# nagadomi/nunif

Hardware: NVIDIA H100
Metric: waifu2x_input_megapixels_per_sec (higher is better)
Workload: dtype f16

## Files before the change

nunif_b200/csrc/gemm_wgmma.cuh:

```cuda
#pragma once
#include "common.cuh"
#include "ptx.cuh"
#include <cuda.h>

namespace nb200 {

enum : int { ACT_NONE = 0, ACT_LRELU01 = 1, ACT_GELU = 2, ACT_RELU = 3 };
enum : int { OUT_NHWC = 0, OUT_PIXSHUF2 = 1, OUT_SPLIT = 2 };

struct GemmParams {
    int B, Ho, Wo, TH, TW, tiles_x, tiles_y;
    int N;
    int taps, cpt;
    int8_t tap_dx[16], tap_dy[16], tap_dyi[16];
    int n_tiles;
    const float* bias;
    int act;
    int out_mode, cout;
    int has_res, res_cy, res_cx;
    int res_before_act;
    int k2;
};

struct GemmMaps {
    CUtensorMap a, b;
    CUtensorMap o[4];
    union {
        CUtensorMap r[4];
        CUtensorMap a2;
    };
};

__device__ __forceinline__ void mbar_init(uint64_t* bar, uint32_t count) {
    asm volatile("mbarrier.init.shared::cta.b64 [%0], %1;" ::"r"(smem_u32(bar)), "r"(count));
}
__device__ __forceinline__ void mbar_expect_tx(uint64_t* bar, uint32_t bytes) {
    asm volatile("mbarrier.arrive.expect_tx.shared::cta.b64 _, [%0], %1;" ::"r"(smem_u32(bar)), "r"(bytes) : "memory");
}
__device__ __forceinline__ void mbar_arrive(uint64_t* bar) {
    asm volatile("mbarrier.arrive.shared::cta.b64 _, [%0];" ::"r"(smem_u32(bar)) : "memory");
}
__device__ __forceinline__ void mbar_wait(uint64_t* bar, uint32_t parity) {
    const uint32_t addr = smem_u32(bar);
    uint32_t done = 0;
#pragma unroll 1
    for (uint32_t it = 0; it < (1u << 18) && !done; ++it)
        asm volatile(
            "{\n\t.reg .pred p;\n\t"
            "mbarrier.try_wait.parity.shared::cta.b64 p, [%1], %2, %3;\n\t"
            "selp.u32 %0, 1, 0, p;\n\t}"
            : "=r"(done) : "r"(addr), "r"(parity), "r"(20000u) : "memory");
    if (!done) __trap();
}
__device__ __forceinline__ void fence_barrier_init() {
    asm volatile("fence.mbarrier_init.release.cluster;" ::: "memory");
    asm volatile("fence.proxy.async.shared::cta;" ::: "memory");
}
__device__ __forceinline__ void tma_load_5d(const CUtensorMap* map, uint64_t* bar, void* dst, int c0, int c1, int c2, int c3, int c4) {
    asm volatile(
        "cp.async.bulk.tensor.5d.shared::cluster.global.tile.mbarrier::complete_tx::bytes [%0], [%1, {%3, %4, %5, %6, %7}], [%2];"
        ::"r"(smem_u32(dst)), "l"(map), "r"(smem_u32(bar)), "r"(c0), "r"(c1), "r"(c2), "r"(c3), "r"(c4) : "memory");
}
__device__ __forceinline__ void tma_load_2d(const CUtensorMap* map, uint64_t* bar, void* dst, int c0, int c1) {
    asm volatile(
        "cp.async.bulk.tensor.2d.shared::cluster.global.tile.mbarrier::complete_tx::bytes [%0], [%1, {%3, %4}], [%2];"
        ::"r"(smem_u32(dst)), "l"(map), "r"(smem_u32(bar)), "r"(c0), "r"(c1) : "memory");
}
__device__ __forceinline__ void tma_load_4d(const CUtensorMap* map, uint64_t* bar, void* dst, int c0, int c1, int c2, int c3) {
    asm volatile(
        "cp.async.bulk.tensor.4d.shared::cluster.global.tile.mbarrier::complete_tx::bytes [%0], [%1, {%3, %4, %5, %6}], [%2];"
        ::"r"(smem_u32(dst)), "l"(map), "r"(smem_u32(bar)), "r"(c0), "r"(c1), "r"(c2), "r"(c3) : "memory");
}
__device__ __forceinline__ void tma_store_4d(const CUtensorMap* map, const void* src, int c0, int c1, int c2, int c3) {
    asm volatile("cp.async.bulk.tensor.4d.global.shared::cta.tile.bulk_group [%0, {%2, %3, %4, %5}], [%1];"
                 ::"l"(map), "r"(smem_u32(src)), "r"(c0), "r"(c1), "r"(c2), "r"(c3) : "memory");
}
__device__ __forceinline__ void tma_store_2d(const CUtensorMap* map, const void* src, int c0, int c1) {
    asm volatile("cp.async.bulk.tensor.2d.global.shared::cta.tile.bulk_group [%0, {%2, %3}], [%1];"
                 ::"l"(map), "r"(smem_u32(src)), "r"(c0), "r"(c1) : "memory");
}
__device__ __forceinline__ void tma_store_commit() { asm volatile("cp.async.bulk.commit_group;" ::: "memory"); }
__device__ __forceinline__ void tma_store_wait_read() { asm volatile("cp.async.bulk.wait_group.read 0;" ::: "memory"); }
__device__ __forceinline__ void fence_async_smem() { asm volatile("fence.proxy.async.shared::cta;" ::: "memory"); }
__device__ __forceinline__ void consumer_bar_sync() { asm volatile("bar.sync 1, 256;" ::: "memory"); }
__device__ __forceinline__ void tma_prefetch_desc(const CUtensorMap* map) {
    asm volatile("prefetch.tensormap [%0];" ::"l"(map) : "memory");
}
__device__ __forceinline__ bool elect_one() {
    uint32_t pred;
    asm volatile(
        "{\n\t.reg .pred p;\n\t"
        "elect.sync _|p, 0xffffffff;\n\t"
        "selp.u32 %0, 1, 0, p;\n\t}"
        : "=r"(pred));
    return pred != 0;
}
__device__ __forceinline__ void wgmma_fence() { asm volatile("wgmma.fence.sync.aligned;" ::: "memory"); }
__device__ __forceinline__ void wgmma_commit() { asm volatile("wgmma.commit_group.sync.aligned;" ::: "memory"); }
template <int N>
__device__ __forceinline__ void wgmma_wait() { asm volatile("wgmma.wait_group.sync.aligned %0;" ::"n"(N) : "memory"); }
template <int K>
__device__ __forceinline__ void wgmma_fence_operands(float (&d)[K]) {
#pragma unroll
    for (int j = 0; j < K; ++j) asm volatile("" : "+f"(d[j])::"memory");
}

template <int SWIZZLE_BYTES>
__device__ __forceinline__ uint64_t make_kmajor_desc(uint32_t saddr) {
    constexpr uint64_t layout = SWIZZLE_BYTES == 128 ? 1 : (SWIZZLE_BYTES == 64 ? 2 : 3);
    constexpr uint64_t sbo = (8 * SWIZZLE_BYTES) >> 4;
    return (uint64_t)((saddr & 0x3FFFF) >> 4) | (1ull << 16) | (sbo << 32) | (layout << 62);
}

template <int N>
__device__ void wgmma_f16(float (&d)[N / 2], uint64_t a, uint64_t b, uint32_t acc);
template <> __device__ __forceinline__ void wgmma_f16<16>(float (&d)[8], uint64_t a, uint64_t b, uint32_t acc) {
    asm volatile("{\n\t.reg .pred p;\n\tsetp.ne.b32 p, %10, 0;\n\t"
                 "wgmma.mma_async.sync.aligned.m64n16k16.f32.f16.f16 {%0, %1, %2, %3, %4, %5, %6, %7}, %8, %9, p, 1, 1, 0, 0;\n\t}"
                 : "+f"(d[0]), "+f"(d[1]), "+f"(d[2]), "+f"(d[3]), "+f"(d[4]), "+f"(d[5]), "+f"(d[6]), "+f"(d[7])
                 : "l"(a), "l"(b), "r"(acc));
}
template <> __device__ __forceinline__ void wgmma_f16<32>(float (&d)[16], uint64_t a, uint64_t b, uint32_t acc) {
    asm volatile("{\n\t.reg .pred p;\n\tsetp.ne.b32 p, %18, 0;\n\t"
                 "wgmma.mma_async.sync.aligned.m64n32k16.f32.f16.f16 {%0, %1, %2, %3, %4, %5, %6, %7, %8, %9, %10, %11, %12, %13, %14, %15}, %16, %17, p, 1, 1, 0, 0;\n\t}"
                 : "+f"(d[0]), "+f"(d[1]), "+f"(d[2]), "+f"(d[3]), "+f"(d[4]), "+f"(d[5]), "+f"(d[6]), "+f"(d[7]), "+f"(d[8]), "+f"(d[9]), "+f"(d[10]), "+f"(d[11]), "+f"(d[12]), "+f"(d[13]), "+f"(d[14]), "+f"(d[15])
                 : "l"(a), "l"(b), "r"(acc));
}
template <> __device__ __forceinline__ void wgmma_f16<48>(float (&d)[24], uint64_t a, uint64_t b, uint32_t acc) {
    asm volatile("{\n\t.reg .pred p;\n\tsetp.ne.b32 p, %26, 0;\n\t"
                 "wgmma.mma_async.sync.aligned.m64n48k16.f32.f16.f16 {%0, %1, %2, %3, %4, %5, %6, %7, %8, %9, %10, %11, %12, %13, %14, %15, %16, %17, %18, %19, %20, %21, %22, %23}, %24, %25, p, 1, 1, 0, 0;\n\t}"
                 : "+f"(d[0]), "+f"(d[1]), "+f"(d[2]), "+f"(d[3]), "+f"(d[4]), "+f"(d[5]), "+f"(d[6]), "+f"(d[7]), "+f"(d[8]), "+f"(d[9]), "+f"(d[10]), "+f"(d[11]), "+f"(d[12]), "+f"(d[13]), "+f"(d[14]), "+f"(d[15]), "+f"(d[16]), "+f"(d[17]), "+f"(d[18]), "+f"(d[19]), "+f"(d[20]), "+f"(d[21]), "+f"(d[22]), "+f"(d[23])
                 : "l"(a), "l"(b), "r"(acc));
}
template <> __device__ __forceinline__ void wgmma_f16<64>(float (&d)[32], uint64_t a, uint64_t b, uint32_t acc) {
    asm volatile("{\n\t.reg .pred p;\n\tsetp.ne.b32 p, %34, 0;\n\t"
                 "wgmma.mma_async.sync.aligned.m64n64k16.f32.f16.f16 {%0, %1, %2, %3, %4, %5, %6, %7, %8, %9, %10, %11, %12, %13, %14, %15, %16, %17, %18, %19, %20, %21, %22, %23, %24, %25, %26, %27, %28, %29, %30, %31}, %32, %33, p, 1, 1, 0, 0;\n\t}"
                 : "+f"(d[0]), "+f"(d[1]), "+f"(d[2]), "+f"(d[3]), "+f"(d[4]), "+f"(d[5]), "+f"(d[6]), "+f"(d[7]), "+f"(d[8]), "+f"(d[9]), "+f"(d[10]), "+f"(d[11]), "+f"(d[12]), "+f"(d[13]), "+f"(d[14]), "+f"(d[15]), "+f"(d[16]), "+f"(d[17]), "+f"(d[18]), "+f"(d[19]), "+f"(d[20]), "+f"(d[21]), "+f"(d[22]), "+f"(d[23]), "+f"(d[24]), "+f"(d[25]), "+f"(d[26]), "+f"(d[27]), "+f"(d[28]), "+f"(d[29]), "+f"(d[30]), "+f"(d[31])
                 : "l"(a), "l"(b), "r"(acc));
}
template <> __device__ __forceinline__ void wgmma_f16<96>(float (&d)[48], uint64_t a, uint64_t b, uint32_t acc) {
    asm volatile("{\n\t.reg .pred p;\n\tsetp.ne.b32 p, %50, 0;\n\t"
                 "wgmma.mma_async.sync.aligned.m64n96k16.f32.f16.f16 {%0, %1, %2, %3, %4, %5, %6, %7, %8, %9, %10, %11, %12, %13, %14, %15, %16, %17, %18, %19, %20, %21, %22, %23, %24, %25, %26, %27, %28, %29, %30, %31, %32, %33, %34, %35, %36, %37, %38, %39, %40, %41, %42, %43, %44, %45, %46, %47}, %48, %49, p, 1, 1, 0, 0;\n\t}"
                 : "+f"(d[0]), "+f"(d[1]), "+f"(d[2]), "+f"(d[3]), "+f"(d[4]), "+f"(d[5]), "+f"(d[6]), "+f"(d[7]), "+f"(d[8]), "+f"(d[9]), "+f"(d[10]), "+f"(d[11]), "+f"(d[12]), "+f"(d[13]), "+f"(d[14]), "+f"(d[15]), "+f"(d[16]), "+f"(d[17]), "+f"(d[18]), "+f"(d[19]), "+f"(d[20]), "+f"(d[21]), "+f"(d[22]), "+f"(d[23]), "+f"(d[24]), "+f"(d[25]), "+f"(d[26]), "+f"(d[27]), "+f"(d[28]), "+f"(d[29]), "+f"(d[30]), "+f"(d[31]), "+f"(d[32]), "+f"(d[33]), "+f"(d[34]), "+f"(d[35]), "+f"(d[36]), "+f"(d[37]), "+f"(d[38]), "+f"(d[39]), "+f"(d[40]), "+f"(d[41]), "+f"(d[42]), "+f"(d[43]), "+f"(d[44]), "+f"(d[45]), "+f"(d[46]), "+f"(d[47])
                 : "l"(a), "l"(b), "r"(acc));
}
template <> __device__ __forceinline__ void wgmma_f16<128>(float (&d)[64], uint64_t a, uint64_t b, uint32_t acc) {
    asm volatile("{\n\t.reg .pred p;\n\tsetp.ne.b32 p, %66, 0;\n\t"
                 "wgmma.mma_async.sync.aligned.m64n128k16.f32.f16.f16 {%0, %1, %2, %3, %4, %5, %6, %7, %8, %9, %10, %11, %12, %13, %14, %15, %16, %17, %18, %19, %20, %21, %22, %23, %24, %25, %26, %27, %28, %29, %30, %31, %32, %33, %34, %35, %36, %37, %38, %39, %40, %41, %42, %43, %44, %45, %46, %47, %48, %49, %50, %51, %52, %53, %54, %55, %56, %57, %58, %59, %60, %61, %62, %63}, %64, %65, p, 1, 1, 0, 0;\n\t}"
                 : "+f"(d[0]), "+f"(d[1]), "+f"(d[2]), "+f"(d[3]), "+f"(d[4]), "+f"(d[5]), "+f"(d[6]), "+f"(d[7]), "+f"(d[8]), "+f"(d[9]), "+f"(d[10]), "+f"(d[11]), "+f"(d[12]), "+f"(d[13]), "+f"(d[14]), "+f"(d[15]), "+f"(d[16]), "+f"(d[17]), "+f"(d[18]), "+f"(d[19]), "+f"(d[20]), "+f"(d[21]), "+f"(d[22]), "+f"(d[23]), "+f"(d[24]), "+f"(d[25]), "+f"(d[26]), "+f"(d[27]), "+f"(d[28]), "+f"(d[29]), "+f"(d[30]), "+f"(d[31]), "+f"(d[32]), "+f"(d[33]), "+f"(d[34]), "+f"(d[35]), "+f"(d[36]), "+f"(d[37]), "+f"(d[38]), "+f"(d[39]), "+f"(d[40]), "+f"(d[41]), "+f"(d[42]), "+f"(d[43]), "+f"(d[44]), "+f"(d[45]), "+f"(d[46]), "+f"(d[47]), "+f"(d[48]), "+f"(d[49]), "+f"(d[50]), "+f"(d[51]), "+f"(d[52]), "+f"(d[53]), "+f"(d[54]), "+f"(d[55]), "+f"(d[56]), "+f"(d[57]), "+f"(d[58]), "+f"(d[59]), "+f"(d[60]), "+f"(d[61]), "+f"(d[62]), "+f"(d[63])
                 : "l"(a), "l"(b), "r"(acc));
}

__device__ __forceinline__ void wgmma_f16_rs96(float (&d)[48], const uint32_t (&a)[4], uint64_t b, uint32_t acc) {
    asm volatile("{\n\t.reg .pred p;\n\tsetp.ne.b32 p, %53, 0;\n\t"
                 "wgmma.mma_async.sync.aligned.m64n96k16.f32.f16.f16 {%0, %1, %2, %3, %4, %5, %6, %7, %8, %9, %10, %11, %12, %13, %14, %15, %16, %17, %18, %19, %20, %21, %22, %23, %24, %25, %26, %27, %28, %29, %30, %31, %32, %33, %34, %35, %36, %37, %38, %39, %40, %41, %42, %43, %44, %45, %46, %47}, {%48, %49, %50, %51}, %52, p, 1, 1, 0;\n\t}"
                 : "+f"(d[0]), "+f"(d[1]), "+f"(d[2]), "+f"(d[3]), "+f"(d[4]), "+f"(d[5]), "+f"(d[6]), "+f"(d[7]), "+f"(d[8]), "+f"(d[9]), "+f"(d[10]), "+f"(d[11]), "+f"(d[12]), "+f"(d[13]), "+f"(d[14]), "+f"(d[15]), "+f"(d[16]), "+f"(d[17]), "+f"(d[18]), "+f"(d[19]), "+f"(d[20]), "+f"(d[21]), "+f"(d[22]), "+f"(d[23]), "+f"(d[24]), "+f"(d[25]), "+f"(d[26]), "+f"(d[27]), "+f"(d[28]), "+f"(d[29]), "+f"(d[30]), "+f"(d[31]), "+f"(d[32]), "+f"(d[33]), "+f"(d[34]), "+f"(d[35]), "+f"(d[36]), "+f"(d[37]), "+f"(d[38]), "+f"(d[39]), "+f"(d[40]), "+f"(d[41]), "+f"(d[42]), "+f"(d[43]), "+f"(d[44]), "+f"(d[45]), "+f"(d[46]), "+f"(d[47])
                 : "r"(a[0]), "r"(a[1]), "r"(a[2]), "r"(a[3]), "l"(b), "r"(acc));
}

__device__ __forceinline__ float gelu_erf(float x) {
    const float a = fabsf(x);
    float q = fmaf(a, 4.88118734e-04f, -7.19881030e-03f);
    q = fmaf(q, a, 5.21468017e-02f);
    q = fmaf(q, a, 4.59595724e-01f);
    q = fmaf(q, a, 1.15100057e+00f);
    const float e = ex2(fmaf(-q, a, -1.0f));
    return fmaxf(x, 0.f) - a * e;
}

template <int K>
__device__ __forceinline__ void apply_act(float (&v)[K], int act) {
    switch (act) {
        case ACT_LRELU01:
#pragma unroll
            for (int j = 0; j < K; ++j) v[j] = v[j] > 0.f ? v[j] : 0.1f * v[j];
            break;
        case ACT_GELU:
#pragma unroll
            for (int j = 0; j < K; ++j) v[j] = gelu_erf(v[j]);
            break;
        case ACT_RELU:
#pragma unroll
            for (int j = 0; j < K; ++j) v[j] = fmaxf(v[j], 0.f);
            break;
        default: break;
    }
}

constexpr int GEMM_CONSUMER_THREADS = 256;
constexpr int GEMM_THREADS = GEMM_CONSUMER_THREADS + 32;

template <int BLOCK_N, int BK>
struct GemmCfg {
    static_assert(BLOCK_N % 16 == 0 && BLOCK_N <= 128, "BLOCK_N: 16..128 (the fp32 accumulators live in registers)");
    static constexpr int SWIZZLE = BK * 2;
    static constexpr int A_BYTES = 128 * BK * 2;
    static constexpr int B_BYTES = BLOCK_N * BK * 2;
    static constexpr int STAGE_BYTES = A_BYTES + ((B_BYTES + 1023) / 1024) * 1024;
    static constexpr int STAGES = (98304 / STAGE_BYTES) < 2 ? 2 : ((98304 / STAGE_BYTES) > 6 ? 6 : (98304 / STAGE_BYTES));
    static constexpr int CW = (BLOCK_N % 64 == 0) ? 64 : ((BLOCK_N % 32 == 0) ? 32 : 16);
    static constexpr int NCH = BLOCK_N / CW;
    static constexpr int CH_BYTES = 128 * CW * 2;
    static_assert(NCH * CH_BYTES <= STAGES * STAGE_BYTES, "epilogue staging must fit in the (drained) pipeline stages");
    static constexpr int SMEM_BYTES = STAGES * STAGE_BYTES + 1024  + 256 ;
};

template <int CW>
__device__ __forceinline__ uint32_t stage_off(int r, int j) {
    if (CW == 64) return (uint32_t)(r * 128 + ((j ^ (r & 7)) << 4));
    if (CW == 32) return (uint32_t)(r * 64 + ((j ^ ((r >> 1) & 3)) << 4));
    return (uint32_t)(r * 32 + ((j ^ ((r >> 2) & 1)) << 4));
}

template <int ROWS>
__device__ __forceinline__ uint32_t sw64_off(int r, int col) {
    return (uint32_t)((col >> 5) * (ROWS * 64)) + stage_off<32>(r, (col & 31) >> 3) + (uint32_t)((col & 7) * 2);
}

template <int BLOCK_N, int BK, bool A2 = false>
// ... 142 lines not shown
```

nunif_b200/csrc/swin_block.cu:

```cuda
#include "gemm_wgmma.cuh"
#include "swin_kernels.h"
#include "tmap.h"
#include <algorithm>

namespace nb200 {

extern int g_tune[16];

constexpr int FM_ROWS = 128, FM_STAGES = 5, FM_THREADS = GEMM_CONSUMER_THREADS + 128;
constexpr int FM_PRODUCER_REGS = 40, FM_CONSUMER_REGS = 232;

template <int C>
struct FmCfg {
    static constexpr int KB = C / 32;
    static constexpr int NBUF = C == 96 ? 3 : 2;
    static constexpr int TILE = FM_ROWS * C * 2;
    static constexpr int STAGE = 128 * C;
    static constexpr int SMEM = NBUF * TILE + FM_STAGES * STAGE + (2 * FM_STAGES + NBUF * (KB + 2) + 1) * 8 + 1024;
    static_assert(SMEM <= 232448, "shared memory per CTA exceeds the opt-in limit");
};

struct FmMaps {
    CUtensorMap x, att, wp, w1, w2, y, wy;
};

template <int K>
__device__ __forceinline__ float (&half96(float (&acc)[K], int h))[48] { return *reinterpret_cast<float(*)[48]>(&acc[48 * h]); }

__device__ __forceinline__ void wgmma_wait_n(int n) {
    if (n == 0) wgmma_wait<0>();
    else wgmma_wait<1>();
}

template <int C, bool PROJ, int CS>
__global__ void __launch_bounds__(FM_THREADS, 1) swin_mlp_fused_kernel(const __grid_constant__ FmMaps maps, const float* __restrict__ bp,
                                                                     const float* __restrict__ b1, const float* __restrict__ b2,
                                                                     const float* __restrict__ by, int ntiles) {
    using Cfg = FmCfg<C>;
    static_assert(CS % 16 == 0 && 2 * C * CS <= Cfg::STAGE && CS * 256 <= Cfg::TILE, "Wy must fit a ring stage, y a tile");
    constexpr int KB = Cfg::KB, NP = (KB + 1) / 2, NH = 2 * C / 64, NHALF = C / 96, NBUF = Cfg::NBUF;
    constexpr int SPT = (PROJ ? NP : 0) + 2 * NH + (CS ? 1 : 0);
    static_assert(SPT > FM_STAGES, "the barrier protocol needs more stages per tile than the ring holds");
    constexpr int XAHEAD = PROJ ? NBUF - 1 : NBUF;
    extern __shared__ uint8_t smem_dyn[];
    uint8_t* smem = smem_dyn + ((1024u - (smem_u32(smem_dyn) & 1023u)) & 1023u);
    uint8_t* ring = smem + NBUF * Cfg::TILE;
    uint64_t* full = reinterpret_cast<uint64_t*>(ring + FM_STAGES * Cfg::STAGE);
    uint64_t* empty = full + FM_STAGES;
    uint64_t* abar = empty + FM_STAGES;
    uint64_t* xbar = abar + NBUF * KB;
    uint64_t* outw = xbar + NBUF;
    uint64_t* xfree = outw + NBUF;
    auto buf = [&](int b) { return smem + b * Cfg::TILE; };
    const int tid = threadIdx.x, warp = tid >> 5;
    const int nt = (ntiles - (int)blockIdx.x + (int)gridDim.x - 1) / (int)gridDim.x;
    if (tid == GEMM_CONSUMER_THREADS) {
        tma_prefetch_desc(&maps.x);
        tma_prefetch_desc(&maps.w1);
        tma_prefetch_desc(&maps.w2);
        if (CS) {
            tma_prefetch_desc(&maps.wy);
            tma_prefetch_desc(&maps.y);
        }
        if (PROJ) {
            tma_prefetch_desc(&maps.att);
            tma_prefetch_desc(&maps.wp);
        }
        for (int s = 0; s < FM_STAGES; ++s) {
            mbar_init(&full[s], 1);
            mbar_init(&empty[s], 2);
        }
        for (int b = 0; b < NBUF; ++b) {
            for (int kb = 0; kb < KB; ++kb) mbar_init(&abar[b * KB + kb], 1);
            mbar_init(&xbar[b], 1);
            mbar_init(&outw[b], 2);
        }
        mbar_init(xfree, 2);
        fence_barrier_init();
    }
    __syncthreads();

    if (warp >= GEMM_CONSUMER_THREADS / 32) {
        asm volatile("setmaxnreg.dec.sync.aligned.u32 %0;" ::"n"(FM_PRODUCER_REGS));
        if (warp == GEMM_CONSUMER_THREADS / 32 && elect_one()) {
            int it = 0;
            auto push = [&](const CUtensorMap* m, int k0, int n0, int rows, int nbox) {
                const int s = it % FM_STAGES;
                mbar_wait(&empty[s], ((it / FM_STAGES) & 1) ^ 1);
                mbar_expect_tx(&full[s], nbox * rows * 64);
                for (int b = 0; b < nbox; ++b) tma_load_2d(m, &full[s], ring + s * Cfg::STAGE + b * rows * 64, k0 + 32 * b, n0);
                ++it;
            };
            for (int j = 0; j < nt; ++j) {
                if (PROJ)
                    for (int p = 0; p < NP; ++p) push(&maps.wp, 64 * p, 0, C, min(2, KB - 2 * p));
                push(&maps.w1, 0, 0, 64, KB);
                for (int hc = 0; hc < NH; ++hc) {
                    if (hc + 1 < NH) push(&maps.w1, 0, (hc + 1) * 64, 64, KB);
                    push(&maps.w2, hc * 64, 0, C, 2);
                }
                if (CS) push(&maps.wy, 0, 0, CS, KB);
            }
        } else if (warp == GEMM_CONSUMER_THREADS / 32 + 1 && elect_one()) {
            auto row = [&](int j) { return ((int)blockIdx.x + j * (int)gridDim.x) * FM_ROWS; };
            auto load_att = [&](int j) {
                const int b = j % NBUF;
                for (int kb = 0; kb < KB; ++kb) {
                    mbar_expect_tx(&abar[b * KB + kb], FM_ROWS * 64);
                    tma_load_2d(&maps.att, &abar[b * KB + kb], buf(b) + kb * (FM_ROWS * 64), kb * 32, row(j));
                }
            };
            auto load_x = [&](int j) {
                uint8_t* dst = buf((j + PROJ) % NBUF);
                mbar_expect_tx(&xbar[j % NBUF], Cfg::TILE);
                for (int kb = 0; kb < KB; ++kb) tma_load_2d(&maps.x, &xbar[j % NBUF], dst + kb * (FM_ROWS * 64), kb * 32, row(j));
            };
            asm volatile("griddepcontrol.wait;" ::: "memory");
            if (PROJ) load_att(0);
            for (int j = 0; j < XAHEAD && j < nt; ++j) load_x(j);
            for (int j = 0; j < nt; ++j) {
                if (PROJ) {
                    mbar_wait(xfree, j & 1);
                    if (j + 1 < nt) load_att(j + 1);
                }
                const int b = j % NBUF;
                mbar_wait(&outw[b], (j / NBUF) & 1);
                if constexpr (CS > 0)
                    for (int c = 0; c < CS / 16; ++c) tma_store_2d(&maps.y, buf(b) + c * (FM_ROWS * 32), 16 * c, row(j));
                else
                    for (int kb = 0; kb < KB; ++kb) tma_store_2d(&maps.x, buf(b) + kb * (FM_ROWS * 64), kb * 32, row(j));
                tma_store_commit();
                tma_store_wait_read();
                if (j + XAHEAD < nt) load_x(j + XAHEAD);
            }
        }
        return;
    }

    asm volatile("setmaxnreg.inc.sync.aligned.u32 %0;" ::"n"(FM_CONSUMER_REGS));
    const int wg = tid >> 7, t = tid & 127;
    const int row0 = wg * 64 + (t >> 5) * 16 + ((t & 31) >> 2);
    const int cq = 2 * (t & 3);
#pragma unroll 1
    for (int it0 = 0; (int)blockIdx.x + it0 / SPT * (int)gridDim.x < ntiles; it0 += SPT) {
        const int j = it0 / SPT;
        int it = it0;
        const int b = j % NBUF;
        const uint32_t par = (j / NBUF) & 1;
        uint8_t* sx1 = buf(b);
        const uint8_t* sxin = buf((j + PROJ) % NBUF);
        const uint32_t x1_base = smem_u32(sx1) + wg * 64 * 64;
        int pending = 0;
        auto take = [&]() -> uint32_t {
            const int s = it % FM_STAGES;
            mbar_wait(&full[s], (it / FM_STAGES) & 1);
            return smem_u32(ring + s * Cfg::STAGE);
        };
        auto commit = [&]() {
            wgmma_commit();
            ++it;
            ++pending;
        };
        auto retire = [&](int n) {
            wgmma_wait_n(n);
#pragma unroll
            for (int k = 0; k < FM_STAGES; ++k)
                if (k < pending - n && t == 0) mbar_arrive(&empty[(it - pending + k) % FM_STAGES]);
            pending = min(pending, n);
        };

        if (PROJ) {
            float acc[C / 2];
#pragma unroll
            for (int i = 0; i < C / 2; ++i) acc[i] = 0.f;
            wgmma_fence_operands(acc);
#pragma unroll
            for (int p = 0; p < NP; ++p) {
                const uint32_t bb = take();
#pragma unroll
                for (int kb = 2 * p; kb < 2 * p + 2 && kb < KB; ++kb) mbar_wait(&abar[b * KB + kb], par);
                wgmma_fence();
#pragma unroll
                for (int kb = 2 * p; kb < 2 * p + 2 && kb < KB; ++kb) {
                    const uint32_t a = x1_base + kb * (FM_ROWS * 64), w = bb + (kb - 2 * p) * (C * 64);
#pragma unroll
                    for (int s = 0; s < 2; ++s)
#pragma unroll
                        for (int h = 0; h < NHALF; ++h)
                            wgmma_f16<96>(half96(acc, h), make_kmajor_desc<64>(a + 32 * s), make_kmajor_desc<64>(w + h * 96 * 64 + 32 * s), 1u);
                }
                commit();
                retire(1);
            }
            retire(0);
            wgmma_fence_operands(acc);
            mbar_wait(&xbar[b], par);
#pragma unroll
            for (int q = 0; q < C / 8; ++q) {
                const int col = 8 * q + cq;
                const float2 bq = __ldg(reinterpret_cast<const float2*>(bp + col));
#pragma unroll
                for (int i = 0; i < 2; ++i) {
                    const uint32_t off = sw64_off<FM_ROWS>(row0 + 8 * i, col);
                    const float2 xv = __half22float2(*reinterpret_cast<const __half2*>(sxin + off));
                    *reinterpret_cast<__half2*>(sx1 + off) =
                        __floats2half2_rn(xv.x + (acc[4 * q + 2 * i] + bq.x), xv.y + (acc[4 * q + 2 * i + 1] + bq.y));
                }
            }
            fence_async_smem();
            asm volatile("bar.sync %0, 128;" ::"r"(2 + wg) : "memory");
            if (t == 0) mbar_arrive(xfree);
        } else {
            mbar_wait(&xbar[b], par);
        }

        float oacc[C / 2];
#pragma unroll
        for (int i = 0; i < C / 2; ++i) oacc[i] = 0.f;
        wgmma_fence_operands(oacc);
        float hacc[2][32];
        uint32_t af[4][4];
        auto fc1 = [&](float (&h)[32]) {
#pragma unroll
            for (int i = 0; i < 32; ++i) h[i] = 0.f;
            wgmma_fence_operands(h);
            const uint32_t bb = take();
            wgmma_fence();
#pragma unroll
            for (int kb = 0; kb < KB; ++kb) {
                const uint32_t a = x1_base + kb * (FM_ROWS * 64), w = bb + kb * (64 * 64);
                wgmma_f16<64>(h, make_kmajor_desc<64>(a), make_kmajor_desc<64>(w), 1u);
                wgmma_f16<64>(h, make_kmajor_desc<64>(a + 32), make_kmajor_desc<64>(w + 32), 1u);
            }
            commit();
        };
        fc1(hacc[0]);
#pragma unroll
        for (int hc = 0; hc < NH; ++hc) {
            const int hb = hc & 1;
            if (hc + 1 < NH) fc1(hacc[hb ^ 1]);
            retire(hc + 1 < NH ? 1 : 0);
            wgmma_fence_operands(hacc[hb]);
#pragma unroll
            for (int kk = 0; kk < 4; ++kk)
#pragma unroll
                for (int q = 0; q < 4; ++q) {
                    const int c8 = 2 * kk + (q >> 1), i = q & 1;
                    const float2 bq = __ldg(reinterpret_cast<const float2*>(b1 + 64 * hc + 8 * c8 + cq));
                    af[kk][q] = pack_half2(gelu_erf(hacc[hb][4 * c8 + 2 * i] + bq.x), gelu_erf(hacc[hb][4 * c8 + 2 * i + 1] + bq.y));
                }
            const uint32_t bb = take();
            wgmma_fence();
#pragma unroll
            for (int kb = 0; kb < 2; ++kb)
#pragma unroll
                for (int s = 0; s < 2; ++s)
#pragma unroll
                    for (int h = 0; h < NHALF; ++h)
                        wgmma_f16_rs96(half96(oacc, h), af[2 * kb + s], make_kmajor_desc<64>(bb + kb * (C * 64) + h * 96 * 64 + 32 * s), 1u);
            commit();
        }
        retire(0);
        wgmma_fence_operands(oacc);
#pragma unroll
        for (int q = 0; q < C / 8; ++q) {
            const int col = 8 * q + cq;
            const float2 bq = __ldg(reinterpret_cast<const float2*>(b2 + col));
#pragma unroll
            for (int i = 0; i < 2; ++i) {
                __half2* p = reinterpret_cast<__half2*>(sx1 + sw64_off<FM_ROWS>(row0 + 8 * i, col));
                const float2 xv = __half22float2(*p);
                *p = __floats2half2_rn(xv.x + (oacc[4 * q + 2 * i] + bq.x), xv.y + (oacc[4 * q + 2 * i + 1] + bq.y));
            }
        }
        fence_async_smem();
        if constexpr (CS > 0) {
            asm volatile("bar.sync %0, 128;" ::"r"(2 + wg) : "memory");
            float yacc[CS / 2];
#pragma unroll
            for (int i = 0; i < CS / 2; ++i) yacc[i] = 0.f;
            wgmma_fence_operands(yacc);
            const uint32_t bb = take();
            wgmma_fence();
#pragma unroll
            for (int kb = 0; kb < KB; ++kb) {
                const uint32_t a = x1_base + kb * (FM_ROWS * 64), w = bb + kb * (CS * 64);
                wgmma_f16<CS>(yacc, make_kmajor_desc<64>(a), make_kmajor_desc<64>(w), 1u);
                wgmma_f16<CS>(yacc, make_kmajor_desc<64>(a + 32), make_kmajor_desc<64>(w + 32), 1u);
            }
            commit();
            retire(0);
            wgmma_fence_operands(yacc);
            consumer_bar_sync();
#pragma unroll
            for (int q = 0; q < CS / 8; ++q) {
                const int col = 8 * q + cq;
                const float2 bq = __ldg(reinterpret_cast<const float2*>(by + col));
#pragma unroll
                for (int i = 0; i < 2; ++i) {
                    __half2* p = reinterpret_cast<__half2*>(sx1 + (col >> 4) * (FM_ROWS * 32) + stage_off<16>(row0 + 8 * i, (col & 15) >> 3) +
                                                            (col & 7) * 2);
                    *p = __floats2half2_rn(yacc[4 * q + 2 * i] + bq.x, yacc[4 * q + 2 * i + 1] + bq.y);
                }
            }
            fence_async_smem();
        }
        asm volatile("bar.sync %0, 128;" ::"r"(2 + wg) : "memory");
        if (t == 0) mbar_arrive(&outw[b]);
    }
}

static int map2d(CUtensorMap* m, const void* base, int cols, long long rows, int box_rows) {
    const cuuint64_t dims[2] = {(cuuint64_t)cols, (cuuint64_t)rows};
    const cuuint64_t strides[1] = {(cuuint64_t)cols * 2};
    const cuuint32_t box[2] = {32, (cuuint32_t)box_rows};
    return encode(m, base, 2, dims, strides, box, 64);
}

template <int C, bool PROJ, int CS = 0>
static int launch_mlp(cudaStream_t st, int ntiles, const FmMaps& maps, const float* bp, const float* b1, const float* b2,
                      const float* by = nullptr) {
    if (ensure_dyn_smem((const void*)swin_mlp_fused_kernel<C, PROJ, CS>, FmCfg<C>::SMEM)) return 1;
    cudaLaunchConfig_t cfg = {};
    int grid = std::min(ntiles, device_sm_count());
    if (g_tune[10] > 0) grid = std::min(grid, g_tune[10]);
    cfg.gridDim = dim3((unsigned)grid); cfg.blockDim = dim3(FM_THREADS); cfg.dynamicSmemBytes = FmCfg<C>::SMEM;
    cfg.stream = st;
    cudaLaunchAttribute at[1];
    at[0].id = cudaLaunchAttributeProgrammaticStreamSerialization;
    at[0].val.programmaticStreamSerializationAllowed = 1;
    cfg.attrs = at; cfg.numAttrs = 1;
    NB_CUDA(cudaLaunchKernelEx(&cfg, swin_mlp_fused_kernel<C, PROJ, CS>, maps, bp, b1, b2, by, ntiles));
    NB_LAUNCHED();
    return 0;
}

int swin_mlp_fused(cudaStream_t st, __half* x, const __half* att, long long T, int C, const __half* wp, const float* bp,
                   const __half* w1, const float* b1, const __half* w2, const float* b2, __half* y, int cs, const __half* wy,
                   const float* by) {
    NB_CHECK(x && w1 && b1 && w2 && b2 && (!att || (wp && bp)) && (!y || (att && wy && by)), "null pointer");
    NB_CHECK(C == 96 || C == 192, "C must be 96 or 192");
    NB_CHECK(!y || (C == 192 && cs == 48) || (C == 96 && cs == 16), "y: cs must be 48 at C = 192 and 16 at C = 96");
    NB_CHECK(T > 0 && T < (1LL << 31), "token count out of range");
    FmMaps maps;
    memset(&maps, 0, sizeof(maps));
    if (map2d(&maps.x, x, C, T, FM_ROWS)) return 1;
    if (att && (map2d(&maps.att, att, C, T, FM_ROWS) || map2d(&maps.wp, wp, C, C, C))) return 1;
    if (map2d(&maps.w1, w1, C, 2 * C, 64) || map2d(&maps.w2, w2, 2 * C, C, C)) return 1;
    if (y) {
        if (map2d(&maps.wy, wy, C, cs, cs)) return 1;
        const cuuint64_t dims[2] = {(cuuint64_t)cs, (cuuint64_t)T};
        const cuuint64_t strides[1] = {(cuuint64_t)cs * 2};
        const cuuint32_t box[2] = {16, FM_ROWS};
        if (encode(&maps.y, y, 2, dims, strides, box, 32)) return 1;
    }
    const double Td = (double)T;
    ProfScope ps(st, PC_FUSED_MLP, Td * C * 2 * (C * ((att ? 1 : 0) + 4) + (y ? cs : 0)), Td * C * 2 * (att ? 2 : 1),
                 Td * (y ? cs : C) * 2);
    const int ntiles = (int)((T + FM_ROWS - 1) / FM_ROWS);
    if (rec_on()) {
        char line[96];
        snprintf(line, sizeof(line), "swin_mlp,%lld,%d,%d,%d", T, C, att ? 1 : 0, y ? cs : 0);
        rec_append(line);
    }
    if (y) return C == 96 ? launch_mlp<96, true, 16>(st, ntiles, maps, bp, b1, b2, by) : launch_mlp<192, true, 48>(st, ntiles, maps, bp, b1, b2, by);
    if (C == 96) return att ? launch_mlp<96, true>(st, ntiles, maps, bp, b1, b2) : launch_mlp<96, false>(st, ntiles, maps, bp, b1, b2);
    return att ? launch_mlp<192, true>(st, ntiles, maps, bp, b1, b2) : launch_mlp<192, false>(st, ntiles, maps, bp, b1, b2);
}

}

using namespace nb200;

extern "C" int nb200_swin_mlp_fused_f16(void* x, const void* att, long long T, int C, const void* wp, const float* bp,
                                        const void* w1, const float* b1, const void* w2, const float* b2, void* stream) {
    return swin_mlp_fused((cudaStream_t)stream, (__half*)x, (const __half*)att, T, C, (const __half*)wp, bp, (const __half*)w1, b1,
                          (const __half*)w2, b2, nullptr, 0, nullptr, nullptr);
}

extern "C" int nb200_swin_mlp_fused_y_f16(void* x, const void* att, long long T, int C, const void* wp, const float* bp,
                                          const void* w1, const float* b1, const void* w2, const float* b2, void* y, int cs,
                                          const void* wy, const float* by, void* stream) {
    NB_CHECK(y, "null pointer");
    return swin_mlp_fused((cudaStream_t)stream, (__half*)x, (const __half*)att, T, C, (const __half*)wp, bp, (const __half*)w1, b1,
                          (const __half*)w2, b2, (__half*)y, cs, (const __half*)wy, by);
}

extern "C" int nb200_swin_attn_fused_f16(const void* x, const void* wqkv, const float* bqkv, const float* bias_table, void* att,
                                         int B, int H, int W, int C, int shift, void* stream) {
    NB_CHECK(bias_table, "null pointer");
    cudaStream_t st = (cudaStream_t)stream;
    float* frag = nullptr;
    NB_CUDA(cudaMallocAsync((void**)&frag, BIAS_FRAG_FLOATS * sizeof(float), st));
    int rc = build_bias_frag(st, bias_table, frag);
    if (!rc) rc = swin_attn_fused(st, (const __half*)x, (const __half*)wqkv, bqkv, frag, (__half*)att, B, H, W, C, shift);
    cudaFreeAsync(frag, st);
    return rc;
}
```

profiles/ab_swin_mlp.py:

```python
#!/usr/bin/env python
import argparse
import ctypes
import json
import os
import re
import statistics
import subprocess
import sys
import tempfile

ROOT = os.path.dirname(os.path.dirname(os.path.abspath(__file__)))
sys.path.insert(0, ROOT)

SHAPES = [(240, 96), (120, 192), (60, 192), (240, 192)]
BATCH = 16
REPS = 7
WINDOW_MS = 60.0
KERNEL_RE = rb"_ZN5nb20021swin_mlp_fused_kernelILi%dE[A-Za-z0-9_]*"


def load(path):
    from nunif_b200 import _lib
    lib = ctypes.CDLL(os.path.abspath(path))
    for name in ("nb200_last_error", "nb200_check_device", "nb200_swin_mlp_fused_f16"):
        res, args = _lib.SIGNATURES[name]
        getattr(lib, name).restype, getattr(lib, name).argtypes = res, args
    return lib


def check(lib, rc):
    if rc != 0:
        raise RuntimeError(lib.nb200_last_error().decode("utf-8", "replace"))


def call(lib, x, w):
    import torch
    att, wp, bp, w1, b1, w2, b2 = w
    B, H, W, C = x.shape
    p = lambda v: ctypes.c_void_p(v.data_ptr())
    check(lib, lib.nb200_swin_mlp_fused_f16(p(x), p(att), B * H * W, C, p(wp), p(bp), p(w1), p(b1), p(w2), p(b2),
                                            ctypes.c_void_p(torch.cuda.current_stream().cuda_stream)))


def inputs(H, C, dev):
    import torch
    g = torch.Generator(device="cpu").manual_seed(H * 1000 + C)
    x = torch.randn(BATCH, H, H, C, generator=g).half().to(dev)
    att = torch.randn(BATCH, H, H, C, generator=g).half().to(dev)
    wp = (0.5 * torch.randn(C, C, generator=g) / C ** 0.5).half().to(dev)
    bp = (0.1 * torch.randn(C, generator=g)).to(dev)
    w1 = (torch.randn(2 * C, C, generator=g) / C ** 0.5).half().to(dev)
    b1 = (0.1 * torch.randn(2 * C, generator=g)).to(dev)
    w2 = (0.05 * torch.randn(C, 2 * C, generator=g) / (2 * C) ** 0.5).half().to(dev)
    b2 = (0.01 * torch.randn(C, generator=g)).to(dev)
    return x, (att, wp, bp, w1, b1, w2, b2)


def window_ms(lib, x, w, n):
    import torch
    e0, e1 = torch.cuda.Event(enable_timing=True), torch.cuda.Event(enable_timing=True)
    e0.record()
    for _ in range(n):
        call(lib, x, w)
    e1.record()
    e1.synchronize()
    return e0.elapsed_time(e1) / n


def launch_smem(libs, dev):
    import torch
    from torch.profiler import ProfilerActivity, profile
    out = {}
    with tempfile.TemporaryDirectory() as d:
        for tag, lib in libs.items():
            for C in (96, 192):
                x, w = inputs(12, C, dev)
                with profile(activities=[ProfilerActivity.CUDA]) as prof:
                    call(lib, x, w)
                    torch.cuda.synchronize()
                path = os.path.join(d, f"{tag}{C}.json")
                prof.export_chrome_trace(path)
                ev = [e for e in json.load(open(path))["traceEvents"]
                      if e.get("cat") == "kernel" and "swin_mlp_fused_kernel" in e.get("name", "")]
                a = ev[0]["args"]
                out[(tag, C)] = (int(a["shared memory"]), int(a["block"][0]))
    return out


def occupancy(so_path, C, smem, threads):
    cuobjdump = os.path.join(os.environ.get("CUDA_HOME", "/usr/local/cuda"), "bin", "cuobjdump")
    with tempfile.TemporaryDirectory() as d:
        subprocess.run([cuobjdump, "-xelf", "all", os.path.abspath(so_path)], cwd=d, check=True, capture_output=True)
        for f in sorted(os.listdir(d)):
            image = open(os.path.join(d, f), "rb").read()
            names = sorted(n for n in set(re.findall(KERNEL_RE % C, image)) if b"_param_" not in n)
            if names:
                break
        else:
            raise RuntimeError(f"swin_mlp_fused_kernel<{C}> not found in {so_path}")
    name = next((n for n in names if b"Lb1E" in n), names[0])
    cu = ctypes.CDLL("libcuda.so.1")

    def ck(rc):
        if rc != 0:
            raise RuntimeError(f"CUDA driver error {rc}")
    mod, fn = ctypes.c_void_p(), ctypes.c_void_p()
    ck(cu.cuModuleLoadData(ctypes.byref(mod), ctypes.c_char_p(image)))
    try:
        ck(cu.cuModuleGetFunction(ctypes.byref(fn), mod, name))
        ck(cu.cuFuncSetAttribute(fn, 8, ctypes.c_int(smem)))
        regs, n = ctypes.c_int(), ctypes.c_int()
        ck(cu.cuFuncGetAttribute(ctypes.byref(regs), 4, fn))
        ck(cu.cuOccupancyMaxActiveBlocksPerMultiprocessor(ctypes.byref(n), fn, threads, ctypes.c_size_t(smem)))
    finally:
        cu.cuModuleUnload(mod)
    return regs.value, n.value


def device_info(index):
    q = subprocess.run(["nvidia-smi", "-i", str(index), "--query-gpu=name,power.limit,clocks.max.sm", "--format=csv,noheader"],
                       capture_output=True, text=True)
    return q.stdout.strip()


def main():
    ap = argparse.ArgumentParser(description=__doc__, formatter_class=argparse.RawDescriptionHelpFormatter)
    ap.add_argument("--base", required=True, help="the build to compare against (libnunif_b200.so)")
    ap.add_argument("--new", default=os.path.join(ROOT, "nunif_b200", "libnunif_b200.so"), help="default: this tree's build")
    ap.add_argument("--out", default=None, help="also write the JSON result here")
    args = ap.parse_args()
    for p in (args.base, args.new):
        if not os.path.isfile(p):
            ap.error(f"no such library: {p}")
    import torch
    from bench import ClockSampler
    if not torch.cuda.is_available():
        raise SystemExit("ab_swin_mlp.py needs a CUDA device")
    dev = torch.device("cuda:0")
    torch.cuda.init()
    torch.zeros(1, device=dev)
    paths = {"base": args.base, "new": args.new}
    libs = {k: load(v) for k, v in paths.items()}
    for lib in libs.values():
        check(lib, lib.nb200_check_device(0))
    info = {"device": torch.cuda.get_device_name(dev), "nvidia_smi": device_info(0), "paths": paths}
    print(f"# {info['device']} | name, power limit, max SM clock: {info['nvidia_smi']}")

    kern = []
    try:
        for (tag, C), (smem, threads) in sorted(launch_smem(libs, dev).items()):
            regs, ctas = occupancy(paths[tag], C, smem, threads)
            kern.append({"build": tag, "C": C, "threads": threads, "regs": regs, "dyn_smem": smem, "ctas_per_sm": ctas})
            print(f"# {tag:4s} swin_mlp_fused_kernel<{C}>: {threads} threads, {regs} registers at launch, {smem} B shared memory/CTA, "
                  f"{ctas} CTA(s)/SM")
    except Exception as e:
        kern.append({"error": f"{type(e).__name__}: {e}"})
        print(f"# occupancy query failed: {type(e).__name__}: {e}")

    rows = []
    with torch.inference_mode(), ClockSampler(0) as clocks:
        for H, C in SHAPES:
            x0, w = inputs(H, C, dev)
            xs = {k: x0.clone() for k in libs}
            for k, lib in libs.items():
                call(lib, xs[k], w)
            torch.cuda.synchronize()
            equal = torch.equal(xs["base"], xs["new"])
            diff = float((xs["base"].float() - xs["new"].float()).abs().max())
            for k, lib in libs.items():
                for _ in range(2):
                    call(lib, xs[k], w)
            est = max(window_ms(libs["base"], xs["base"], w, 2), window_ms(libs["new"], xs["new"], w, 2))
            n = max(3, int(WINDOW_MS / max(est, 1e-3)))
            ms = {k: [] for k in libs}
            for r in range(REPS):
                for k in (("base", "new") if r % 2 == 0 else ("new", "base")):
                    ms[k].append(window_ms(libs[k], xs[k], w, n))
            row = {"B": BATCH, "H": H, "W": H, "C": C, "calls_per_window": n, "equal": equal, "max_abs_diff": diff}
            for k in libs:
                row[k] = {"median_ms": statistics.median(ms[k]), "min_ms": min(ms[k]), "max_ms": max(ms[k])}
            row["new_over_base"] = row["new"]["median_ms"] / row["base"]["median_ms"]
            rows.append(row)
            b, nw = row["base"], row["new"]
            print(f"{BATCH}x{H}x{H}x{C}: base {b['median_ms']:.4f} ms [{b['min_ms']:.4f}, {b['max_ms']:.4f}]  "
                  f"new {nw['median_ms']:.4f} ms [{nw['min_ms']:.4f}, {nw['max_ms']:.4f}]  new/base {row['new_over_base']:.3f}  "
                  f"outputs {'identical' if equal else f'DIFFER (max |d| {diff:g})'}", flush=True)
            del xs, x0, w
    result = {"info": info, "clocks": clocks.summary(), "kernels": kern, "shapes": rows,
              "all_equal": all(r["equal"] for r in rows)}
    print(json.dumps(result))
    if args.out:
        os.makedirs(os.path.dirname(os.path.abspath(args.out)), exist_ok=True)
        with open(args.out, "w") as fh:
            json.dump(result, fh, indent=1)
    return 0 if result["all_equal"] else 1


if __name__ == "__main__":
    sys.exit(main())
```

Measured before the change: 80.91.

## Read residual x directly from global into registers for C=192 projection path

For the PROJ path with two buffers and no side output (C=192), the kernel stops staging the residual input x through shared memory via TMA. Consumers now load x from global (L2-prefetched by the producer) into registers while the projection GEMM retires. This frees the x buffer so attention tiles can be loaded two tiles ahead and drops the xfree handshake. The cost is extra register pressure and uncoalesced-ish global loads in the consumer, plus a consumer-side griddepcontrol.wait. The A/B script also gains a CS path and a grid-cap sweep.

Measured after the change: 81.52 (median of 6 runs). Within noise of the previous version (+0.8%).

```diff
diff --git a/nunif_b200/csrc/gemm_wgmma.cuh b/nunif_b200/csrc/gemm_wgmma.cuh
--- a/nunif_b200/csrc/gemm_wgmma.cuh
+++ b/nunif_b200/csrc/gemm_wgmma.cuh
@@ -65,6 +65,9 @@
     asm volatile(
         "cp.async.bulk.tensor.2d.shared::cluster.global.tile.mbarrier::complete_tx::bytes [%0], [%1, {%3, %4}], [%2];"
         ::"r"(smem_u32(dst)), "l"(map), "r"(smem_u32(bar)), "r"(c0), "r"(c1) : "memory");
+}
+__device__ __forceinline__ void tma_prefetch_l2_2d(const CUtensorMap* map, int c0, int c1) {
+    asm volatile("cp.async.bulk.prefetch.tensor.2d.L2.global.tile [%0, {%1, %2}];" ::"l"(map), "r"(c0), "r"(c1) : "memory");
 }
 __device__ __forceinline__ void tma_load_4d(const CUtensorMap* map, uint64_t* bar, void* dst, int c0, int c1, int c2, int c3) {
     asm volatile(
diff --git a/nunif_b200/csrc/swin_block.cu b/nunif_b200/csrc/swin_block.cu
--- a/nunif_b200/csrc/swin_block.cu
+++ b/nunif_b200/csrc/swin_block.cu
@@ -35,13 +35,15 @@
 template <int C, bool PROJ, int CS>
 __global__ void __launch_bounds__(FM_THREADS, 1) swin_mlp_fused_kernel(const __grid_constant__ FmMaps maps, const float* __restrict__ bp,
                                                                      const float* __restrict__ b1, const float* __restrict__ b2,
-                                                                     const float* __restrict__ by, int ntiles) {
+                                                                     const float* __restrict__ by, const __half* xg, int T,
+                                                                     int ntiles) {
     using Cfg = FmCfg<C>;
     static_assert(CS % 16 == 0 && 2 * C * CS <= Cfg::STAGE && CS * 256 <= Cfg::TILE, "Wy must fit a ring stage, y a tile");
     constexpr int KB = Cfg::KB, NP = (KB + 1) / 2, NH = 2 * C / 64, NHALF = C / 96, NBUF = Cfg::NBUF;
     constexpr int SPT = (PROJ ? NP : 0) + 2 * NH + (CS ? 1 : 0);
     static_assert(SPT > FM_STAGES, "the barrier protocol needs more stages per tile than the ring holds");
-    constexpr int XAHEAD = PROJ ? NBUF - 1 : NBUF;
+    constexpr bool XG = PROJ && NBUF == 2 && CS == 0;
+    constexpr int XAHEAD = XG ? 0 : PROJ ? NBUF - 1 : NBUF;
     extern __shared__ uint8_t smem_dyn[];
     uint8_t* smem = smem_dyn + ((1024u - (smem_u32(smem_dyn) & 1023u)) & 1023u);
     uint8_t* ring = smem + NBUF * Cfg::TILE;
@@ -109,6 +111,8 @@
                     mbar_expect_tx(&abar[b * KB + kb], FM_ROWS * 64);
                     tma_load_2d(&maps.att, &abar[b * KB + kb], buf(b) + kb * (FM_ROWS * 64), kb * 32, row(j));
                 }
+                if (XG)
+                    for (int kb = 0; kb < KB; ++kb) tma_prefetch_l2_2d(&maps.x, kb * 32, row(j));
             };
             auto load_x = [&](int j) {
                 uint8_t* dst = buf((j + PROJ) % NBUF);
@@ -116,10 +120,13 @@
                 for (int kb = 0; kb < KB; ++kb) tma_load_2d(&maps.x, &xbar[j % NBUF], dst + kb * (FM_ROWS * 64), kb * 32, row(j));
             };
             asm volatile("griddepcontrol.wait;" ::: "memory");
-            if (PROJ) load_att(0);
+            if (XG)
+                for (int j = 0; j < NBUF && j < nt; ++j) load_att(j);
+            else if (PROJ)
+                load_att(0);
             for (int j = 0; j < XAHEAD && j < nt; ++j) load_x(j);
             for (int j = 0; j < nt; ++j) {
-                if (PROJ) {
+                if (PROJ && !XG) {
                     mbar_wait(xfree, j & 1);
                     if (j + 1 < nt) load_att(j + 1);
                 }
@@ -131,7 +138,8 @@
                     for (int kb = 0; kb < KB; ++kb) tma_store_2d(&maps.x, buf(b) + kb * (FM_ROWS * 64), kb * 32, row(j));
                 tma_store_commit();
                 tma_store_wait_read();
-                if (j + XAHEAD < nt) load_x(j + XAHEAD);
+                if (XG && j + NBUF < nt) load_att(j + NBUF);
+                if (!XG && j + XAHEAD < nt) load_x(j + XAHEAD);
             }
         }
         return;
@@ -141,6 +149,7 @@
     const int wg = tid >> 7, t = tid & 127;
     const int row0 = wg * 64 + (t >> 5) * 16 + ((t & 31) >> 2);
     const int cq = 2 * (t & 3);
+    if (XG) asm volatile("griddepcontrol.wait;" ::: "memory");
 #pragma unroll 1
     for (int it0 = 0; (int)blockIdx.x + it0 / SPT * (int)gridDim.x < ntiles; it0 += SPT) {
         const int j = it0 / SPT;
@@ -192,9 +201,20 @@
                 commit();
                 retire(1);
             }
+            uint32_t xr[XG ? C / 8 : 1][2];
+            if (XG) {
+                const int r = ((int)blockIdx.x + j * (int)gridDim.x) * FM_ROWS + row0;
+#pragma unroll
+                for (int i = 0; i < 2; ++i) {
+                    const __half* xp = xg + (size_t)(r + 8 * i) * C + cq;
+                    const bool in = r + 8 * i < T;
+#pragma unroll
+                    for (int q = 0; q < (XG ? C / 8 : 0); ++q) xr[q][i] = in ? *reinterpret_cast<const uint32_t*>(xp + 8 * q) : 0u;
+                }
+            }
             retire(0);
             wgmma_fence_operands(acc);
-            mbar_wait(&xbar[b], par);
+            if (!XG) mbar_wait(&xbar[b], par);
 #pragma unroll
             for (int q = 0; q < C / 8; ++q) {
                 const int col = 8 * q + cq;
@@ -202,14 +222,15 @@
 #pragma unroll
                 for (int i = 0; i < 2; ++i) {
                     const uint32_t off = sw64_off<FM_ROWS>(row0 + 8 * i, col);
-                    const float2 xv = __half22float2(*reinterpret_cast<const __half2*>(sxin + off));
+                    const float2 xv = __half22float2(XG ? *reinterpret_cast<const __half2*>(&xr[XG ? q : 0][i])
+                                                        : *reinterpret_cast<const __half2*>(sxin + off));
                     *reinterpret_cast<__half2*>(sx1 + off) =
                         __floats2half2_rn(xv.x + (acc[4 * q + 2 * i] + bq.x), xv.y + (acc[4 * q + 2 * i + 1] + bq.y));
                 }
             }
             fence_async_smem();
             asm volatile("bar.sync %0, 128;" ::"r"(2 + wg) : "memory");
-            if (t == 0) mbar_arrive(xfree);
+            if (!XG && t == 0) mbar_arrive(xfree);
         } else {
             mbar_wait(&xbar[b], par);
         }
@@ -318,8 +339,8 @@
 }
 
 template <int C, bool PROJ, int CS = 0>
-static int launch_mlp(cudaStream_t st, int ntiles, const FmMaps& maps, const float* bp, const float* b1, const float* b2,
-                      const float* by = nullptr) {
+static int launch_mlp(cudaStream_t st, const __half* x, int T, int ntiles, const FmMaps& maps, const float* bp, const float* b1,
+                      const float* b2, const float* by = nullptr) {
     if (ensure_dyn_smem((const void*)swin_mlp_fused_kernel<C, PROJ, CS>, FmCfg<C>::SMEM)) return 1;
     cudaLaunchConfig_t cfg = {};
     int grid = std::min(ntiles, device_sm_count());
@@ -330,7 +351,7 @@
     at[0].id = cudaLaunchAttributeProgrammaticStreamSerialization;
     at[0].val.programmaticStreamSerializationAllowed = 1;
     cfg.attrs = at; cfg.numAttrs = 1;
-    NB_CUDA(cudaLaunchKernelEx(&cfg, swin_mlp_fused_kernel<C, PROJ, CS>, maps, bp, b1, b2, by, ntiles));
+    NB_CUDA(cudaLaunchKernelEx(&cfg, swin_mlp_fused_kernel<C, PROJ, CS>, maps, bp, b1, b2, by, (const __half*)x, T, ntiles));
     NB_LAUNCHED();
     return 0;
 }
@@ -363,9 +384,13 @@
         snprintf(line, sizeof(line), "swin_mlp,%lld,%d,%d,%d", T, C, att ? 1 : 0, y ? cs : 0);
         rec_append(line);
     }
-    if (y) return C == 96 ? launch_mlp<96, true, 16>(st, ntiles, maps, bp, b1, b2, by) : launch_mlp<192, true, 48>(st, ntiles, maps, bp, b1, b2, by);
-    if (C == 96) return att ? launch_mlp<96, true>(st, ntiles, maps, bp, b1, b2) : launch_mlp<96, false>(st, ntiles, maps, bp, b1, b2);
-    return att ? launch_mlp<192, true>(st, ntiles, maps, bp, b1, b2) : launch_mlp<192, false>(st, ntiles, maps, bp, b1, b2);
+    const int Ti = (int)T;
+    if (y)
+        return C == 96 ? launch_mlp<96, true, 16>(st, x, Ti, ntiles, maps, bp, b1, b2, by)
+                       : launch_mlp<192, true, 48>(st, x, Ti, ntiles, maps, bp, b1, b2, by);
+    if (C == 96)
+        return att ? launch_mlp<96, true>(st, x, Ti, ntiles, maps, bp, b1, b2) : launch_mlp<96, false>(st, x, Ti, ntiles, maps, bp, b1, b2);
+    return att ? launch_mlp<192, true>(st, x, Ti, ntiles, maps, bp, b1, b2) : launch_mlp<192, false>(st, x, Ti, ntiles, maps, bp, b1, b2);
 }
 
 }
diff --git a/profiles/ab_swin_mlp.py b/profiles/ab_swin_mlp.py
--- a/profiles/ab_swin_mlp.py
+++ b/profiles/ab_swin_mlp.py
@@ -12,7 +12,7 @@
 ROOT = os.path.dirname(os.path.dirname(os.path.abspath(__file__)))
 sys.path.insert(0, ROOT)
 
-SHAPES = [(240, 96), (120, 192), (60, 192), (240, 192)]
+SHAPES = [(240, 96, 0), (120, 192, 0), (60, 192, 0), (240, 192, 0), (240, 192, 48)]
 BATCH = 16
 REPS = 7
 WINDOW_MS = 60.0
@@ -22,7 +22,7 @@
 def load(path):
     from nunif_b200 import _lib
     lib = ctypes.CDLL(os.path.abspath(path))
-    for name in ("nb200_last_error", "nb200_check_device", "nb200_swin_mlp_fused_f16"):
+    for name in ("nb200_last_error", "nb200_check_device", "nb200_swin_mlp_fused_f16", "nb200_swin_mlp_fused_y_f16", "nb200_tune_set"):
         res, args = _lib.SIGNATURES[name]
         getattr(lib, name).restype, getattr(lib, name).argtypes = res, args
     return lib
@@ -35,14 +35,23 @@
 
 def call(lib, x, w):
     import torch
-    att, wp, bp, w1, b1, w2, b2 = w
+    att, wp, bp, w1, b1, w2, b2 = w[:7]
     B, H, W, C = x.shape
     p = lambda v: ctypes.c_void_p(v.data_ptr())
-    check(lib, lib.nb200_swin_mlp_fused_f16(p(x), p(att), B * H * W, C, p(wp), p(bp), p(w1), p(b1), p(w2), p(b2),
-                                            ctypes.c_void_p(torch.cuda.current_stream().cuda_stream)))
-
-
-def inputs(H, C, dev):
+    st = ctypes.c_void_p(torch.cuda.current_stream().cuda_stream)
+    if len(w) > 7:
+        y, wy, by = w[7:]
+        check(lib, lib.nb200_swin_mlp_fused_y_f16(p(x), p(att), B * H * W, C, p(wp), p(bp), p(w1), p(b1), p(w2), p(b2), p(y),
+                                                  wy.shape[0], p(wy), p(by), st))
+    else:
+        check(lib, lib.nb200_swin_mlp_fused_f16(p(x), p(att), B * H * W, C, p(wp), p(bp), p(w1), p(b1), p(w2), p(b2), st))
+
+
+def output(x, w):
+    return w[7] if len(w) > 7 else x
+
+
+def inputs(H, C, dev, cs=0):
     import torch
     g = torch.Generator(device="cpu").manual_seed(H * 1000 + C)
     x = torch.randn(BATCH, H, H, C, generator=g).half().to(dev)
@@ -53,7 +62,12 @@
     b1 = (0.1 * torch.randn(2 * C, generator=g)).to(dev)
     w2 = (0.05 * torch.randn(C, 2 * C, generator=g) / (2 * C) ** 0.5).half().to(dev)
     b2 = (0.01 * torch.randn(C, generator=g)).to(dev)
-    return x, (att, wp, bp, w1, b1, w2, b2)
+    if not cs:
+        return x, (att, wp, bp, w1, b1, w2, b2)
+    wy = (torch.randn(cs, C, generator=g) / C ** 0.5).half().to(dev)
+    by = torch.randn(cs, generator=g).to(dev)
+    y = torch.empty(BATCH * H * H, cs, dtype=torch.float16, device=dev)
+    return x, (att, wp, bp, w1, b1, w2, b2, y, wy, by)
 
 
 def window_ms(lib, x, w, n):
@@ -123,13 +137,50 @@
     return q.stdout.strip()
 
 
+def cap_sweep(lib, caps, dev):
+    import torch
+    rows = []
+    for H, C, cs in SHAPES:
+        x, w = inputs(H, C, dev, cs)
+        tiles = (BATCH * H * H + 127) // 128
+        ms = {cap: [] for cap in caps}
+        try:
+            n = None
+            for cap in caps:
+                check(lib, lib.nb200_tune_set(10, cap))
+                for _ in range(2):
+                    call(lib, x, w)
+                n = n or max(3, int(WINDOW_MS / max(window_ms(lib, x, w, 2), 1e-3)))
+            for r in range(REPS):
+                for cap in (caps if r % 2 == 0 else caps[::-1]):
+                    check(lib, lib.nb200_tune_set(10, cap))
+                    ms[cap].append(window_ms(lib, x, w, n))
+        finally:
+            lib.nb200_tune_set(10, 0)
+        for cap in caps:
+            grid = min(tiles, cap)
+            med = statistics.median(ms[cap])
+            row = {"B": BATCH, "H": H, "W": H, "C": C, "CS": cs, "cap": cap, "grid": grid, "tiles": tiles,
+                   "median_ms": med, "min_ms": min(ms[cap]), "max_ms": max(ms[cap]), "us_per_tile_per_cta": 1e3 * med * grid / tiles}
+            rows.append(row)
+            print(f"{BATCH}x{H}x{H}x{C}{f' CS {cs}' if cs else ''} cap {cap:4d}: {med:.4f} ms [{row['min_ms']:.4f}, "
+                  f"{row['max_ms']:.4f}]  {row['us_per_tile_per_cta']:.2f} us per tile per CTA "
+                  f"({row['us_per_tile_per_cta'] / rows[-1 - caps.index(cap)]['us_per_tile_per_cta']:.3f}x cap {caps[0]})", flush=True)
+        del x, w
+    return rows
+
+
 def main():
     ap = argparse.ArgumentParser(description=__doc__, formatter_class=argparse.RawDescriptionHelpFormatter)
-    ap.add_argument("--base", required=True, help="the build to compare against (libnunif_b200.so)")
+    ap.add_argument("--base", default=None, help="the build to compare against (libnunif_b200.so)")
     ap.add_argument("--new", default=os.path.join(ROOT, "nunif_b200", "libnunif_b200.so"), help="default: this tree's build")
+    ap.add_argument("--caps", default=None, help="comma-separated grid caps: time --new alone at each (no --base)")
     ap.add_argument("--out", default=None, help="also write the JSON result here")
     args = ap.parse_args()
-    for p in (args.base, args.new):
+    if (args.base is None) == (args.caps is None):
+        ap.error("give either --base or --caps")
+    paths = {"new": args.new} if args.caps else {"base": args.base, "new": args.new}
+    for p in paths.values():
         if not os.path.isfile(p):
             ap.error(f"no such library: {p}")
     import torch
@@ -139,12 +190,23 @@
     dev = torch.device("cuda:0")
     torch.cuda.init()
     torch.zeros(1, device=dev)
-    paths = {"base": args.base, "new": args.new}
     libs = {k: load(v) for k, v in paths.items()}
     for lib in libs.values():
         check(lib, lib.nb200_check_device(0))
     info = {"device": torch.cuda.get_device_name(dev), "nvidia_smi": device_info(0), "paths": paths}
     print(f"# {info['device']} | name, power limit, max SM clock: {info['nvidia_smi']}")
+
+    if args.caps:
+        caps = [int(c) for c in args.caps.split(",")]
+        with torch.inference_mode(), ClockSampler(0) as clocks:
+            rows = cap_sweep(libs["new"], caps, dev)
+        result = {"info": info, "clocks": clocks.summary(), "caps": rows}
+        print(json.dumps(result))
+        if args.out:
+            os.makedirs(os.path.dirname(os.path.abspath(args.out)), exist_ok=True)
+            with open(args.out, "w") as fh:
+                json.dump(result, fh, indent=1)
+        return 0
 
     kern = []
     try:
@@ -159,33 +221,35 @@
 
     rows = []
     with torch.inference_mode(), ClockSampler(0) as clocks:
-        for H, C in SHAPES:
-            x0, w = inputs(H, C, dev)
+        for H, C, cs in SHAPES:
+            x0, w = inputs(H, C, dev, cs)
             xs = {k: x0.clone() for k in libs}
+            ws = {k: w[:7] + (torch.empty_like(w[7]),) + w[8:] if cs else w for k in libs}
             for k, lib in libs.items():
-                call(lib, xs[k], w)
+                call(lib, xs[k], ws[k])
             torch.cuda.synchronize()
-            equal = torch.equal(xs["base"], xs["new"])
-            diff = float((xs["base"].float() - xs["new"].float()).abs().max())
+            outs = {k: output(xs[k], ws[k]) for k in libs}
+            equal = torch.equal(outs["base"], outs["new"]) and (not cs or torch.equal(xs["base"], xs["new"]))
+            diff = float((outs["base"].float() - outs["new"].float()).abs().max())
             for k, lib in libs.items():
                 for _ in range(2):
-                    call(lib, xs[k], w)
-            est = max(window_ms(libs["base"], xs["base"], w, 2), window_ms(libs["new"], xs["new"], w, 2))
+                    call(lib, xs[k], ws[k])
+            est = max(window_ms(libs["base"], xs["base"], ws["base"], 2), window_ms(libs["new"], xs["new"], ws["new"], 2))
             n = max(3, int(WINDOW_MS / max(est, 1e-3)))
             ms = {k: [] for k in libs}
             for r in range(REPS):
                 for k in (("base", "new") if r % 2 == 0 else ("new", "base")):
-                    ms[k].append(window_ms(libs[k], xs[k], w, n))
-            row = {"B": BATCH, "H": H, "W": H, "C": C, "calls_per_window": n, "equal": equal, "max_abs_diff": diff}
+                    ms[k].append(window_ms(libs[k], xs[k], ws[k], n))
+            row = {"B": BATCH, "H": H, "W": H, "C": C, "CS": cs, "calls_per_window": n, "equal": equal, "max_abs_diff": diff}
             for k in libs:
                 row[k] = {"median_ms": statistics.median(ms[k]), "min_ms": min(ms[k]), "max_ms": max(ms[k])}
             row["new_over_base"] = row["new"]["median_ms"] / row["base"]["median_ms"]
             rows.append(row)
             b, nw = row["base"], row["new"]
-            print(f"{BATCH}x{H}x{H}x{C}: base {b['median_ms']:.4f} ms [{b['min_ms']:.4f}, {b['max_ms']:.4f}]  "
+            print(f"{BATCH}x{H}x{H}x{C}{f' CS {cs}' if cs else ''}: base {b['median_ms']:.4f} ms [{b['min_ms']:.4f}, {b['max_ms']:.4f}]  "
                   f"new {nw['median_ms']:.4f} ms [{nw['min_ms']:.4f}, {nw['max_ms']:.4f}]  new/base {row['new_over_base']:.3f}  "
                   f"outputs {'identical' if equal else f'DIFFER (max |d| {diff:g})'}", flush=True)
-            del xs, x0, w
+            del xs, ws, x0, w
     result = {"info": info, "clocks": clocks.summary(), "kernels": kern, "shapes": rows,
               "all_equal": all(r["equal"] for r in rows)}
     print(json.dumps(result))
```
